# AlexZou14/Wave-Mamba

Hardware: AMD Instinct MI355X
Metric: UHD (3840x2160) images/sec fwd (higher is better)
Workload: dtype f32; 1 GPU; Wave-Mamba UHD-LL inference config (wf=32, n_l=[1,2,4], n_h=[1,1,2]), 1x3x2160x3840 reflect-padded to 2176x3840, seeded random init, one image per GPU per step, replicas (no collective); one forward at a time, its down-path high-frequency branches on side streams: True

## Files before the change

include/wavemamba_hip.h:

```cpp
#ifndef WAVEMAMBA_HIP_H
#define WAVEMAMBA_HIP_H

#include <stddef.h>
#include <stdint.h>

#ifdef __cplusplus
extern "C" {
#endif

#define WM_OK 0
#define WM_EINVAL (-1)
#define WM_ENULL (-2)
#define WM_EALIGN (-3)
#define WM_EWORKSPACE (-4)
#define WM_EUNSUPPORTED (-5)
#define WM_EHIP (-6)

#define WM_F32 0
#define WM_BF16 1

int wm_abi_version(void);
const char* wm_build_id(void);
const char* wm_strerror(int code);

// ... 55 lines not shown
                    const float* skip_scale2, float* out, int out_nchw, int B, int64_t L, int C, int plane_dtype,
                    void* stream);
int wm_lfss_in_conv_fwd(const float* tok, int tok_nchw, const float* ln_w, const float* ln_b, float ln_eps,
                        const float* in_proj_weight, const float* conv_weight, const float* conv_bias, float* xc,
                        int B, int H, int W, int C, int plane_dtype, void* stream);
int wm_lfss_in_conv_band_rows(int B, int H, int W);
int wm_lfss_out_conv_fwd(const void* f, const float* conv2_weight, const float* conv2_bias, const float* tok1,
                         const float* conv3_weight, const float* conv3_bias, const float* skip_scale2, float* out,
                         int out_nchw, int B, int H, int W, int C, int plane_dtype, void* stream);
int wm_lfss_mid_rz_tok_fwd(const void* ysum, int ny, int64_t ystride, const float* tok, int tok_nchw, const float* ln1_w,
                           const float* ln1_b, float ln1_eps, const float* in_proj_weight, const float* out_norm_w,
                           const float* out_norm_b, float out_norm_eps, const float* out_proj_weight, const float* skip_scale,
                           float* tok1, int B, int64_t L, int C, int plane_dtype, void* stream);
int wm_lfss_ffn_fwd(const float* tok1, const float* ln2_w, const float* ln2_b, float ln2_eps, const float* conv1_weight,
                    const float* conv1_bias, const float* conv2_weight, const float* conv2_bias, const float* conv3_weight,
                    const float* conv3_bias, const float* skip_scale2, float* out, int out_nchw, int B, int H, int W, int C,
                    int plane_dtype, int band_rows, void* stream);
int wm_lfss_ffn_band_rows(int B, int H, int W);

int wm_layernorm2d_fwd(const float* x, const float* weight, const float* bias, float eps, float* y,
                       int B, int64_t L, int C, void* stream);

size_t wm_gram_workspace_bytes(int B, int C, int64_t L);
int wm_gram_fwd(const float* X, const float* Y, float* G, float* nx, float* ny, void* workspace,
                size_t workspace_bytes, int B, int C, int64_t L, void* stream);

int wm_dwconv3x3_wgrad(const float* x, const float* gy, float* dW, float* db, int B, int C, int H, int W,
                       void* stream);
int wm_layernorm2d_bwd(const float* x, const float* weight, const float* gy, float eps, float* gx,
                       float* dweight, float* dbias, int B, int64_t L, int C, void* stream);


int wm_conv2d_select(int mode);
size_t wm_conv2d_wfrag_bytes(int Cout, int Cin, int ks);
int wm_conv2d_prep(const float* weight, void* wfrag, int Cout, int Cin, int ks, void* stream);
int wm_conv2d_ln_fwd(const float* x, const float* ln_weight, const float* ln_bias, float ln_eps, const void* wfrag, const float* bias,
                     const float* residual, float* y, int B, int Cin, int Cout, int H, int W, void* stream);
int wm_dwconv_conv1x1_fwd(const float* x, int64_t x_batch_stride, const float* dw_weight, const float* dw_bias, int act,
                          const void* wfrag, const float* bias, const float* residual, float* y, int B, int C, int Cout, int H,
                          int W, void* stream);
int wm_ln_conv1x1_dwconv_fwd(const float* x, const float* ln_weight, const float* ln_bias, float ln_eps, const void* wfrag,
                             const float* bias, const float* dw_weight, const float* dw_bias, float* y, int B, int Cin, int Cout,
                             int Cdw, int H, int W, int band_rows, void* stream);
int wm_conv2d_f16_steps(const float* x, const float* weight, const float* bias, float* y, float* amax, void* wfrag, int B, int Cin,
                        int Cout, int H, int W, int ks, int dgrad, void* stream);
int wm_conv2d_fwd(const float* xa, const float* xb, const int* xb_index, const void* wfrag, const float* bias,
                  const float* gate, const float* residual, float* y, int B, int Ca, int Cb, int Cb_src, int Cout,
                  int H, int W, int ks, void* stream);
int wm_conv2d_gated_fwd(const float* xa, const float* xb, const int* xb_index, const void* wfrag3, const void* wfrag1,
                        const float* bias1, float* y, int B, int Ca, int Cb, int Cb_src, int Cout, int H, int W,
                        void* stream);
int wm_conv2d_dwt_fwd(const void* img, const void* wfrag, const float* bias, void* ll, void* hl, void* lh, void* hh, int B, int Cin,
                      int Cout, int H, int W, int dtype, void* stream);
int wm_idwt_conv2d_fwd(const void* low, const void* high, const void* wfrag, const float* bias, const float* residual, float* y, int B,
                       int Cin, int Cout, int H, int W, int dtype, void* stream);

size_t wm_ss2d_core_bwd_workspace_bytes(int B, int D, int H, int W, int N, int R);
int wm_ss2d_core_bwd(const float* x, const float* x_proj_weight, const float* dt_projs_weight,
                     const float* dt_projs_bias, const float* A_logs, const float* Ds, const float* dy_row_fwd,
                     const float* dy_row_rev, const float* dy_col_fwd, const float* dy_col_rev, float* dx,
                     float* dx_proj_weight, float* ddt_projs_weight, float* ddt_projs_bias, float* dA_logs, float* dDs,
                     void* workspace, size_t workspace_bytes, int B, int D, int H, int W, int N, int R, void* stream);

int wm_layernorm_tok_fwd(const float* x, const float* weight, const float* bias, float eps, float* y, int64_t T, int C,
                         void* stream);
int wm_layernorm_tok_bwd(const float* x, const float* weight, const float* gy, float eps, float* gx, float* dweight,
// ... 90 lines not shown
```

wave_mamba_amd/_lib.py:

```python
import ctypes
import os

HERE = os.path.dirname(os.path.abspath(__file__))
LIB_PATH = os.environ.get("WAVEMAMBA_HIP_LIB") or os.path.join(HERE, "libwavemamba_hip.so")

WM_F32, WM_BF16 = 0, 1
WM_OK, WM_EINVAL, WM_ENULL, WM_EALIGN, WM_EWORKSPACE, WM_EUNSUPPORTED, WM_EHIP = 0, -1, -2, -3, -4, -5, -6
WM_PROF_NKERNELS = 20
ABI_VERSION = 34

_c = ctypes
_p, _i, _i64, _sz = _c.c_void_p, _c.c_int, _c.c_int64, _c.c_size_t

SIGNATURES = {
    "wm_abi_version": (_i, []),
    "wm_build_id": (_c.c_char_p, []),
    "wm_strerror": (_c.c_char_p, [_i]),
    "wm_dwt2d_fwd": (_i, [_p] * 5 + [_i] * 5 + [_p]),
    "wm_dwt2d_bwd": (_i, [_p] * 5 + [_i] * 5 + [_p]),
    "wm_idwt2d_fwd": (_i, [_p] * 4 + [_i64] * 4 + [_p] + [_i] * 5 + [_p]),
    "wm_idwt2d_bwd": (_i, [_p] * 5 + [_i64] * 4 + [_i] * 5 + [_p]),
    "wm_selscan_fwd_workspace_bytes": (_sz, [_i] * 5),
    "wm_selscan_fwd": (_i, [_p] * 10 + [_p, _sz] + [_i] * 6 + [_p]),
    "wm_selscan_bwd_workspace_bytes": (_sz, [_i] * 5),
# ... 31 lines not shown
    "wm_paired_patches_u8": (_i, [_p, _p, _p, _i, _i, _i, _p]),
    "wm_linear_wgrad": (_i, [_p, _p, _p, _i64, _i, _i, _p]),
    "wm_conv2d_wgrad_workspace_bytes": (_sz, [_i] * 6),
    "wm_conv2d_wgrad": (_i, [_p, _p, _p, _p, _p, _sz] + [_i] * 6 + [_p]),
    "wm_plane_sums": (_i, [_p, _p, _i, _i, _i, _i, _p]),
    "wm_psnr_ssim_y_workspace_bytes": (_sz, [_i] * 4),
    "wm_psnr_ssim_y_u8": (_i, [_p, _p] + [_i64] * 4 + [_i] * 5 + [_p, _p, _sz, _p]),
    "wm_y_channel_u8": (_i, [_p] + [_i64] * 4 + [_i] * 4 + [_p, _p]),
    "wm_l1_mean_fwd": (_i, [_p, _p, _p, _i64, _p]),
    "wm_l1_mean_bwd": (_i, [_p, _p, _p, _p, _i64, _p]),
    "wm_ssim_workspace_bytes": (_sz, [_i64, _i, _i]),
    "wm_ssim_mean_fwd": (_i, [_p] * 8 + [_sz, _i64, _i, _i, _p]),
    "wm_ssim_mean_bwd": (_i, [_p] * 7 + [_i64, _i, _i, _p]),
    "wm_gate_fwd": (_i, [_p] * 3 + [_i, _i] + [_i64] * 4 + [_p]),
    "wm_gate_bwd": (_i, [_p] * 5 + [_i, _i] + [_i64] * 6 + [_p]),
    "wm_scale_add_fwd": (_i, [_p] * 4 + [_i, _i, _i64, _p]),
    "wm_scale_add_bwd": (_i, [_p] * 5 + [_i, _i, _i64, _p]),
    "wm_match_index": (_i, [_p, _p, _p, _p, _i, _i, _p]),
    "wm_attn_fold": (_i, [_p] * 6 + [_i, _i, _i, _p]),
    "wm_skff_workspace_bytes": (_sz, [_i, _i]),
    "wm_skff_fwd": (_i, [_p] * 7 + [_p, _sz] + [_i] * 5 + [_p]),
    "wm_conv2d_wfrag_bytes": (_sz, [_i, _i, _i]),
    "wm_conv2d_prep": (_i, [_p, _p, _i, _i, _i, _p]),
    "wm_conv2d_fwd": (_i, [_p] * 8 + [_i] * 8 + [_p]),
    "wm_conv2d_ln_fwd": (_i, [_p, _p, _p, _c.c_float, _p, _p, _p, _p] + [_i] * 5 + [_p]),
    "wm_dwconv_conv1x1_fwd": (_i, [_p, _i64, _p, _p, _i, _p, _p, _p, _p] + [_i] * 5 + [_p]),
    "wm_ln_conv1x1_dwconv_fwd": (_i, [_p, _p, _p, _c.c_float, _p, _p, _p, _p, _p] + [_i] * 7 + [_p]),
    "wm_patchify_conv_fwd": (_i, [_p] * 4 + [_i] * 6 + [_p]),
    "wm_conv2d_f16_steps": (_i, [_p] * 6 + [_i] * 7 + [_p]),
    "wm_conv2d_gated_fwd": (_i, [_p] * 7 + [_i] * 7 + [_p]),
    "wm_conv2d_dwt_fwd": (_i, [_p] * 7 + [_i] * 6 + [_p]),
    "wm_idwt_conv2d_fwd": (_i, [_p] * 6 + [_i] * 6 + [_p]),
    "wm_conv2d_select": (_i, [_i]),
    "wm_prof_enable": (None, [ctypes.c_uint]),
    "wm_prof_collect": (_i, [_c.POINTER(_i), _c.POINTER(_c.c_double)]),
    "wm_event_synchronize_relaxed": (_i, [_p]),
    "wm_zero_arena_register": (_i, [_p, _c.c_size_t]),
    "wm_zero_arena_unregister": (_i, [_p]),
    "wm_dwconv3x3_wgrad_det_workspace_bytes": (_sz, [_i] * 4),
    "wm_dwconv3x3_wgrad_det": (_i, [_p] * 4 + [_p, _sz] + [_i] * 4 + [_p]),
    "wm_layernorm2d_bwd_det_workspace_bytes": (_sz, [_i, _i64, _i]),
    "wm_layernorm2d_bwd_det": (_i, [_p, _p, _p, _c.c_float, _p, _p, _p, _p, _sz, _i, _i64, _i, _p]),
    "wm_layernorm_tok_bwd_det_workspace_bytes": (_sz, [_i64, _i]),
    "wm_layernorm_tok_bwd_det": (_i, [_p, _p, _p, _c.c_float, _p, _p, _p, _p, _sz, _i64, _i, _p]),
    "wm_linear_wgrad_det_workspace_bytes": (_sz, [_i64, _i, _i]),
    "wm_linear_wgrad_det": (_i, [_p, _p, _p, _p, _sz, _i64, _i, _i, _p]),
    "wm_plane_sums_det_workspace_bytes": (_sz, [_i] * 4),
    "wm_plane_sums_det": (_i, [_p, _p, _p, _sz, _i, _i, _i, _i, _p]),
    "wm_scale_add_bwd_det_workspace_bytes": (_sz, [_i, _i, _i64]),
    "wm_scale_add_bwd_det": (_i, [_p] * 5 + [_p, _sz, _i, _i, _i64, _p]),
    "wm_l1_mean_fwd_det_workspace_bytes": (_sz, [_i64]),
    "wm_l1_mean_fwd_det": (_i, [_p, _p, _p, _p, _sz, _i64, _p]),
    "wm_selscan_bwd_det_workspace_bytes": (_sz, [_i] * 5),
    "wm_selscan_bwd_det": (_i, [_p] * 15 + [_p, _sz] + [_i] * 6 + [_p]),
    "wm_channel_gather_fwd": (_i, [_p, _p, _p, _i, _i, _i, _i64, _p]),
    "wm_channel_gather_bwd": (_i, [_p, _p, _p, _i, _i, _i, _i64, _p]),
}

_lib = None


class WaveMambaHipError(RuntimeError):
    pass


def load():
# ... 36 lines not shown
```

wave_mamba_amd/csrc/conv.hip:

```cpp
#include "host_common.h"
#include "conv2d.hip.h"
#include "conv2d_ws.hip.h"
#include "patchify.hip.h"
#include "dw_pw.hip.h"
#include "pw_dw.hip.h"

using namespace wm;

static Conv2dArgs conv_args(const void* xa, int Ca, const void* wfrag, const float* bias, void* y, int Cout, int H, int W) {
    Conv2dArgs a;
    a.xa = (const float*)xa; a.wfrag = (const uint4*)wfrag; a.bias = bias; a.y = (float*)y;
    a.Ca = Ca; a.Cout = Cout; a.H = H; a.W = W;
    a.nch = (Ca + 15) / 16; a.mtot = (Cout + 31) / 32;
    return a;
}

static int conv_tail_check(int B, int H, int W, const void* wfrag) {
    if (B > 65535 || (long long)H * W >= (1ll << 31)) return WM_EUNSUPPORTED;
    if (!aligned16(wfrag)) return WM_EALIGN;
    return WM_OK;
}

template <int KS, int RW, int MT, bool G1X1 = false, bool F16 = false, bool LNIN = false>
static int conv2d_launch(const wm::Conv2dArgs& a, int B, hipStream_t st) {
// ... 11 lines not shown
}

#ifndef WM_CONV_WS_RW2
#define WM_CONV_WS_RW2 4
#endif
#ifndef WM_CONV_WS_RW1
#define WM_CONV_WS_RW1 4
#endif
#ifndef WM_CONV_WS_RWG
#define WM_CONV_WS_RWG 2
#endif
#ifndef WM_CONV_WS_NPW1
#define WM_CONV_WS_NPW1 4
#endif
#ifndef WM_CONV_RW1
#define WM_CONV_RW1 3
#endif
static std::atomic<int> g_conv_select{0};
static int conv_select_mode() { return g_conv_select.load(std::memory_order_relaxed); }
static long long conv_ws_ntiles(const wm::Conv2dArgs& a, int B, int th) {
    return (long long)B * ((a.W + wm::kWsTW - 1) / wm::kWsTW) * ((a.H + th - 1) / th);
}
static bool conv_ws_enabled(const wm::Conv2dArgs& a, int B, int th) {
    const int mode = conv_select_mode();
    if (mode == 1) return false;
    const long long cmax = std::max(std::max(a.Ca, a.xb ? a.Cbsrc : 0), a.Cout);
    if (cmax * a.H * a.W * 4 >= (1ll << 32) || (a.xb_idx && a.Cb > 128)) return false;
    if (a.gate && a.res) return false;
    if (mode == 2) return true;
    if ((a.gate || a.res) && a.mtot > 1) return false;
    return conv_ws_ntiles(a, B, th) >= 768;
}

template <int RW, int MT, bool G1X1 = false, bool EPI = false, int NPW = 4, bool F16 = false, bool DWTE = false, bool IWTI = false>
static int conv2d_ws_launch(const wm::Conv2dArgs& a, int B, hipStream_t st) {
    using Cfg = wm::ConvWsCfg<RW, MT, G1X1, NPW>;
    static bool configured[64] = {};
    int ncu = 0;
    int rc = wm::lds_optin((const void*)wm::conv3x3_ws_kernel<RW, MT, G1X1, EPI, NPW, F16, DWTE, IWTI>, Cfg::LDS_BYTES, configured);
    if (!rc) rc = wm::device_cus(&ncu);
    if (rc) return rc;
    const long long ntiles = conv_ws_ntiles(a, B, Cfg::TH);
    if (ntiles >= (1ll << 31)) return WM_EUNSUPPORTED;
    const int cus = std::max(8, ncu & ~7);
    const int G = (int)std::min<long long>(cus, ((ntiles + 7) / 8) * 8);
    hipLaunchKernelGGL((wm::conv3x3_ws_kernel<RW, MT, G1X1, EPI, NPW, F16, DWTE, IWTI>), dim3((unsigned)G), dim3(256 + 64 * NPW), Cfg::LDS_BYTES, st, a, B);
    return launch_status();
}

template <bool F16, bool LNIN>
static int conv2d_walk(wm::Conv2dArgs& a, int B, int ks, hipStream_t st) {
    for (int mb = 0, n; mb < a.mtot; mb += n) {
        a.mbase = mb;
        const int left = a.mtot - mb;
        int rc = WM_EUNSUPPORTED;
        n = 1;
        if (LNIN || ks == 1) {
            if (left >= 3) { rc = conv2d_launch<1, 2, 3, false, F16, LNIN>(a, B, st); n = 3; }
            else if (left == 2) { rc = conv2d_launch<1, 4, 2, false, F16, LNIN>(a, B, st); n = 2; }
            else rc = conv2d_launch<1, 4, 1, false, F16, LNIN>(a, B, st);
        } else if constexpr (!LNIN) {
            if (conv_ws_enabled(a, B, 8)) {
                const bool epi = !F16 && (a.gate || a.res);
                if (epi) { if constexpr (!F16) rc = conv2d_ws_launch<WM_CONV_WS_RW1, 1, false, true>(a, B, st); }
                else if (left >= 2) { rc = conv2d_ws_launch<WM_CONV_WS_RW2, 2, false, false, 4, F16>(a, B, st); n = 2; }
                else rc = conv2d_ws_launch<WM_CONV_WS_RW1, 1, false, false, WM_CONV_WS_NPW1, F16>(a, B, st);
            } else if (left >= 2) { rc = conv2d_launch<3, 4, 2, false, F16>(a, B, st); n = 2; }
            else rc = conv2d_launch<3, WM_CONV_RW1, 1, false, F16>(a, B, st);
        }
        if (rc) return rc;
    }
    return WM_OK;
}

extern "C" {

int wm_patchify_conv_fwd(const float* img, const float* weight, const float* bias, float* y, int B, int Cin, int Cout, int H, int W,
                         int r, void* stream) {
    if (B < 0 || Cin <= 0 || Cout <= 0 || H < 0 || W < 0) return WM_EINVAL;
    if (r != 2 && r != 4 && r != 8) return WM_EUNSUPPORTED;
    if (H % r || W % r) return WM_EINVAL;
    if (Cout != 16 && Cout != 32 && Cout != 48 && Cout != 64) return WM_EUNSUPPORTED;
    const size_t lds = (size_t)Cin * r * r * Cout * sizeof(float);
    if (lds > 64 * 1024) return WM_EUNSUPPORTED;
    if (B == 0 || H == 0 || W == 0) return WM_OK;
    if (!img || !weight || !y) return WM_ENULL;
    if (!aligned16(img)) return WM_EALIGN;
    if ((long long)B * Cin * H * W >= (1ll << 40)) return WM_EUNSUPPORTED;
    const int Ho = H / r, Wo = W / r;
    const int spr = (Wo + 255) / 256;
    const long long nsegs = (long long)B * Ho * spr;
    const int spb = (int)((nsegs + 4095) / 4096);
    const long long blocks = (nsegs + spb - 1) / spb;
    hipStream_t st = (hipStream_t)stream;
    ProfScope ps(18, st);
#define WM_PF(R, CO) hipLaunchKernelGGL((patchify_conv_kernel<R, CO>), dim3((unsigned)blocks), dim3(256), lds, st, img, weight, bias, y, \
                                        B, Cin, H, W, spr, nsegs, spb)
#define WM_PFR(R) do { if (Cout == 16) WM_PF(R, 16); else if (Cout == 32) WM_PF(R, 32); else if (Cout == 48) WM_PF(R, 48); else WM_PF(R, 64); } while (0)
    if (r == 2) WM_PFR(2); else if (r == 4) WM_PFR(4); else WM_PFR(8);
// ... 135 lines not shown
    if (ks != 1 && ks != 3) return WM_EUNSUPPORTED;
    if (wm_conv2d_wfrag_bytes(Cout, Cin, ks) == 0) return WM_EUNSUPPORTED;
    if (B == 0 || H == 0 || W == 0) return WM_OK;
    if (!x || !weight || !y || !amax || !wfrag) return WM_ENULL;
    if (!aligned16(wfrag)) return WM_EALIGN;
    hipStream_t st = (hipStream_t)stream;
    if (zero_out(amax, 2 * sizeof(float), st) != hipSuccess) return WM_EHIP;
    const long long nx = (long long)B * Cin * H * W, nw = (long long)Cout * Cin * ks * ks;
    long long blocks = (nx / 4 + 256 * 8 - 1) / (256 * 8);
    blocks = blocks < 1 ? 1 : (blocks > 512 ? 512 : blocks);
    const int nch = (Cin + 15) / 16, mtot = (Cout + 31) / 32;
    const long long items = (long long)nch * ks * ks * mtot * 128;
    const int nprep = (int)(items <= 512 ? 1 : (items >= 32 * 512 ? 32 : (items + 511) / 512));
    hipLaunchKernelGGL(cv_amax_prep_kernel, dim3((unsigned)blocks + nprep), dim3(256), 0, st, x, nx, weight, nw, (unsigned*)amax,
                       (uint4*)wfrag, Cout, Cin, ks * ks, nch, mtot, dgrad ? 1 : 0, nprep);
    int rc = launch_status();
    if (rc) return rc;
    return conv2d_fwd_f16(x, wfrag, amax, bias, y, B, Cin, Cout, H, W, ks, stream);
}

int wm_conv2d_dwt_fwd(const void* img, const void* wfrag, const float* bias, void* ll, void* hl, void* lh, void* hh, int B, int Cin,
                      int Cout, int H, int W, int dtype, void* stream) {
    if (B < 0 || Cin <= 0 || Cout <= 0 || H < 0 || W < 0) return WM_EINVAL;
    if (H % 2 || W % 2) return WM_EINVAL;
    if (dtype != WM_F32 || Cout != 32) return WM_EUNSUPPORTED;
    if (B == 0 || H == 0 || W == 0) return WM_OK;
    if (!img || !wfrag || !ll || !hl || !lh || !hh) return WM_ENULL;
    if (const int rc = conv_tail_check(B, H, W, wfrag)) return rc;
    hipStream_t st = (hipStream_t)stream;
    Conv2dArgs a = conv_args(img, Cin, wfrag, bias, ll, Cout, H, W);
    a.yband[0] = (float*)hl; a.yband[1] = (float*)lh; a.yband[2] = (float*)hh;
    if (conv_select_mode() == 1 || (long long)std::max(Cin, Cout) * H * W * 4 >= (1ll << 32)) return WM_EUNSUPPORTED;
    ProfScope ps(13, st);
    return conv2d_ws_launch<WM_CONV_WS_RW1, 1, false, false, WM_CONV_WS_NPW1, false, true>(a, B, st);
}

int wm_idwt_conv2d_fwd(const void* low, const void* high, const void* wfrag, const float* bias, const float* residual, float* y, int B,
                       int Cin, int Cout, int H, int W, int dtype, void* stream) {
    if (B < 0 || Cin <= 0 || Cout <= 0 || H < 0 || W < 0) return WM_EINVAL;
    if (H % 2 || W % 2) return WM_EINVAL;
    if (dtype != WM_F32 || Cin != 32) return WM_EUNSUPPORTED;
    if (B == 0 || H == 0 || W == 0) return WM_OK;
    if (!low || !high || !wfrag || !y) return WM_ENULL;
    if (const int rc = conv_tail_check(B, H, W, wfrag)) return rc;
    hipStream_t st = (hipStream_t)stream;
    Conv2dArgs a = conv_args(low, Cin, wfrag, bias, y, Cout, H, W);
    a.xb = (const float*)high; a.Cbsrc = 3 * Cin;
    a.res = residual;
    if (conv_select_mode() == 1 || (long long)std::max(Cin, Cout) * H * W * 4 >= (1ll << 32)) return WM_EUNSUPPORTED;
    ProfScope ps(13, st);
    for (int mb = 0; mb < a.mtot; ++mb) {
        a.mbase = mb;
        const int rc = residual ? conv2d_ws_launch<WM_CONV_WS_RW1, 1, false, true, 4, false, false, true>(a, B, st)
                                : conv2d_ws_launch<WM_CONV_WS_RW1, 1, false, false, WM_CONV_WS_NPW1, false, false, true>(a, B, st);
        if (rc) return rc;
    }
    return WM_OK;
}

int wm_conv2d_gated_fwd(const float* xa, const float* xb, const int* xb_index, const void* wfrag3, const void* wfrag1,
                        const float* bias1, float* y, int B, int Ca, int Cb, int Cb_src, int Cout, int H, int W,
                        void* stream) {
    if (B < 0 || Ca <= 0 || Cb < 0 || Cout <= 0 || H < 0 || W < 0 || Cb_src < 0) return WM_EINVAL;
    if (B == 0 || H == 0 || W == 0) return WM_OK;
    if (!xa || !wfrag3 || !wfrag1 || !y || (Cb > 0 && !xb)) return WM_ENULL;
    if (Cb > 0 && Ca % 8 != 0) return WM_EUNSUPPORTED;
    if (Cb > 0 && !xb_index && Cb_src != Cb) return WM_EINVAL;
    if (const int rc = conv_tail_check(B, H, W, wfrag3)) return rc;
    if (!aligned16(wfrag1)) return WM_EALIGN;
    hipStream_t st = (hipStream_t)stream;
    Conv2dArgs a = conv_args(xa, Ca, wfrag3, nullptr, y, Cout, H, W);
    if (Cb > 0) { a.xb = xb; a.xb_idx = xb_index; }
    a.Cb = Cb; a.Cbsrc = Cb_src; a.nch = (Ca + Cb + 15) / 16;
    a.wfrag1 = (const uint4*)wfrag1; a.bias1 = bias1;
    ProfScope ps(13, st);
    for (int mb = 0; mb < a.mtot;) {
        a.mbase = mb;
        int rc;
        const bool two = a.mtot - mb >= 2;
        if (conv_ws_enabled(a, B, two ? 2 * WM_CONV_WS_RWG : 8)) {
            if (two) { rc = conv2d_ws_launch<WM_CONV_WS_RWG, 2, true>(a, B, st); mb += 2; }
            else { rc = conv2d_ws_launch<4, 1, true>(a, B, st); mb += 1; }
        } else if (a.mtot - mb >= 2) { rc = conv2d_launch<3, 2, 2, true>(a, B, st); mb += 2; }
        else { rc = conv2d_launch<3, 4, 1, true>(a, B, st); mb += 1; }
        if (rc) return rc;
    }
    return WM_OK;
}

int wm_conv2d_select(int mode) {
    if (mode < 0 || mode > 2) return WM_EINVAL;
    g_conv_select.store(mode, std::memory_order_relaxed);
    return WM_OK;
}

#if WM_CV_STAMP
int wm_debug_conv_stamps(unsigned long long* out) {
    return (int)hipMemcpyFromSymbol(out, HIP_SYMBOL(wm::g_cv_stamps), sizeof(unsigned long long) * 2 * 128 * 8);
}
#endif

}
```

wave_mamba_amd/csrc/conv2d_ws.hip.h:

```cpp
#pragma once
#include <type_traits>
#include "conv2d.hip.h"
#include "haar.hip.h"

namespace wm {

constexpr int kWsTW = 64;

template <int RW, int MT, bool G1X1, int NPW = 4>
struct ConvWsCfg {
    static constexpr int NPT = 64 * NPW;
    static constexpr int PW = kWsTW + 2;
    static constexpr int TH = 2 * RW;
    static constexpr int NPIX = (TH + 2) * PW;
    static constexpr int PIT = (NPIX + NPT - 1) / NPT;
    static constexpr int W_ITEMS = 9 * MT * 2 * 64;
    static constexpr int W1_ITEMS = G1X1 ? MT * 2 * 64 : 0;
    static constexpr int BUF_ITEMS = 4 * NPIX + W_ITEMS + W1_ITEMS;
    static constexpr int LDS_BYTES = 2 * BUF_ITEMS * 16 + 2 * MT * 32 * 4;
};

struct ConvWsTiles {
    int tiles_x, ntiles_img, first, stride, count;
    __device__ ConvWsTiles(int B, int H, int W, int TH, int g, int G) {
        tiles_x = (W + kWsTW - 1) / kWsTW;
        ntiles_img = tiles_x * ((H + TH - 1) / TH);
        const int ntiles = ntiles_img * B, nper = (ntiles + 7) / 8;
        const int x = g & 7, slot = g >> 3;
        stride = G >> 3;
        first = x * nper + slot;
        const int end = min((x + 1) * nper, ntiles);
        count = first < end ? (end - first + stride - 1) / stride : 0;
    }
    __device__ void locate(int j, int TH, int& b, int& h0, int& w0) const {
        const int t = first + j * stride;
        b = t / ntiles_img;
        const int ti = t - b * ntiles_img;
        h0 = (ti / tiles_x) * TH;
        w0 = (ti % tiles_x) * kWsTW;
    }
};

#ifndef WM_CV_STAMP
#define WM_CV_STAMP 0
#endif
#if WM_CV_STAMP
__device__ unsigned long long g_cv_stamps[2 * 128 * 8];
#define CV_STAMP(role, it, k) do { if (WM_CV_STAMP && blockIdx.x == 0 && lane == 0 && (wave & 3) == 0 && (it) < 128) \
        g_cv_stamps[((role) * 128 + (it)) * 8 + (k)] = __builtin_readcyclecounter(); } while (0)
#else
#define CV_STAMP(role, it, k) do { } while (0)
#endif

using u32x4_t = __attribute__((ext_vector_type(4))) unsigned;
template <int OFF>
__device__ __forceinline__ void ws_lds_store16(unsigned addr, const uint4& v) {
    u32x4_t d = {v.x, v.y, v.z, v.w};
    asm volatile("ds_write_b128 %0, %1 offset:%2" : : "v"(addr), "v"(d), "n"(OFF) : "memory");
}

__device__ __forceinline__ void ws_barrier_lds() { asm volatile("s_waitcnt lgkmcnt(0)\n\ts_barrier" ::: "memory"); }

__device__ __forceinline__ float ws_from_pair_lane(float v) {
    return __builtin_bit_cast(float, __builtin_amdgcn_update_dpp(0, __builtin_bit_cast(int, v), 0xB1, 0xf, 0xf, false));
}

template <int RW, int MT, bool G1X1, bool EPI, int NPW = 4, bool F16 = false, bool DWTE = false, bool IWTI = false>
__global__ __launch_bounds__(256 + 64 * NPW, (4 + NPW) / 4) void conv3x3_ws_kernel(const Conv2dArgs a, const int B) {
    extern __shared__ __attribute__((aligned(16))) unsigned char cv_smem[];
    static_assert(!(F16 && G1X1), "the fp16 form (conv2d.hip.h) serves the plain convolutions of the training step");
    static_assert(!DWTE || (MT == 1 && !G1X1 && !EPI && !F16 && RW % 2 == 0), "the analysis epilogue: one plain 32-channel row tile, whole quads per wave");
    static_assert(!IWTI || (!G1X1 && !F16), "the synthesis staging: the plain bf16 form");
    const float sx = F16 ? cv_pow2_scale(a.amax[0]) : 1.0f;
    const float osc = F16 ? 1.0f / (sx * cv_pow2_scale(a.amax[1])) : 1.0f;
    using Cfg = ConvWsCfg<RW, MT, G1X1, NPW>;
    constexpr int PW = Cfg::PW, TH = Cfg::TH, NPIX = Cfg::NPIX, PIT = Cfg::PIT, NPT = Cfg::NPT;
    constexpr int W_ITEMS = Cfg::W_ITEMS, W1_ITEMS = Cfg::W1_ITEMS, BUF = Cfg::BUF_ITEMS;
    uint4* const smem = reinterpret_cast<uint4*>(cv_smem);

    const int tid = threadIdx.x, lane = tid & 63;
    const int wave = __builtin_amdgcn_readfirstlane(tid >> 6);
    const ConvWsTiles tl(B, a.H, a.W, TH, (int)blockIdx.x, (int)gridDim.x);
    if (tl.count == 0) return;
    const int nch = a.nch;
    const int n_it = tl.count * nch;
    const int H = a.H, W = a.W;
    const long long HW = (long long)H * W;

    if (tid < 2 * MT * 32) {
        const int which = tid / (MT * 32), ch = a.mbase * 32 + tid % (MT * 32);
        const float* src = which ? a.bias1 : a.bias;
        reinterpret_cast<float*>(smem + 2 * BUF)[tid] = (src && ch < a.Cout) ? src[ch] : 0.0f;
    }
    if (wave >= 4) {
        const int ptid = tid - 256, pw = wave - 4;
        const unsigned lds_base = (unsigned)(size_t)(__attribute__((address_space(3))) unsigned char*)cv_smem;
        static_assert(2 * NPIX * 16 < 65536, "the lo plane sits within the ds_write offset field");
        constexpr int QR = (TH + 4) / 2, QC = (kWsTW + 4) / 2;
        static_assert(!IWTI || QR * QC <= NPT, "one quad per producer thread");
        constexpr int PSL = IWTI ? 4 : PIT;
        const int qr = IWTI ? ptid / QC : 0, qc = IWTI ? ptid - qr * QC : 0;
        const int h2 = IWTI ? a.H >> 1 : 0, w2 = IWTI ? a.W >> 1 : 0;
        const unsigned HW2b = IWTI ? (unsigned)(h2 * w2) * 4u : 0u;
        float pin[2][2][PSL][8];
        unsigned okm[2][PIT];
        int ccs[2] = {0, 0};
        unsigned poff[PIT];
        unsigned okF[PIT];
        int jf = -1, ccf = nch - 1;
        const float* xaF = a.xa;
        const float* xbF = a.xa;
        int idxv0 = 0, idxv1 = 0, bF = -1;

        auto fetch_w = [&](int buf, int cc) {
            uint4* s_w = smem + buf * BUF + 4 * NPIX;
            const uint4* wsrc = a.wfrag + ((long long)cc * 9 * a.mtot) * 128;
            constexpr int W_IT = (W_ITEMS + NPT - 1) / NPT;
#pragma unroll
            for (int it = 0; it < W_IT; ++it) {
                const int item0 = it * NPT + pw * 64;
                if (W_ITEMS % NPT == 0 || item0 < W_ITEMS) {
                    const int tm = item0 >> 7, tap = tm / MT, m = tm - tap * MT;
                    const uint4* g = wsrc + (tap * a.mtot + a.mbase + m) * 128 + (item0 & 64) + lane;
                    __builtin_amdgcn_global_load_lds((const __attribute__((address_space(1))) void*)g,
                                                     (__attribute__((address_space(3))) void*)(s_w + item0), 16, 0, 0);
                }
            }
            if constexpr (G1X1) {
// ... 143 lines not shown
            ws_barrier_lds();
            CV_STAMP(1, i, 4);
        };

        advance(); fetch_half(C0{}, C0{}); fetch_half(C0{}, C1{});
        fetch_w(0, ccs[0]);
        if (n_it > 1) { advance(); fetch_half(C1{}, C0{}); fetch_half(C1{}, C1{}); }
        stage_half(C0{}, C0{}, 0); stage_half(C0{}, C1{}, 0);
        __builtin_amdgcn_s_waitcnt(0x0070);
        ws_barrier_lds();
        for (int i = 0; i < n_it; i += 2) {
            step(C0{}, C1{}, i + 2 < n_it, i + 1 < n_it, 1, i);
            if (i + 1 >= n_it) break;
            step(C1{}, C0{}, i + 3 < n_it, i + 2 < n_it, 0, i + 1);
        }
        return;
    }

    f32x16_t acc[MT][RW];
    f32x16_t acc1[G1X1 ? MT : 1][G1X1 ? RW : 1];
    auto zero_acc = [&](auto MC) {
        constexpr int m = decltype(MC)::value;
#pragma unroll
        for (int r = 0; r < RW; ++r)
#pragma unroll
            for (int i = 0; i < 16; ++i) { acc[m][r][i] = 0.0f; if (G1X1) acc1[m][r][i] = 0.0f; }
    };
    using M0 = std::integral_constant<int, 0>;
    using M1 = std::integral_constant<int, MT - 1>;
    static_assert(MT <= 2, "at most two row tiles per launch");
    zero_acc(M0{});
    if (MT > 1) zero_acc(M1{});
    const int khalf = lane >> 5, px = lane & 31;
    const int cw = wave & 1, rg = wave >> 1;

    const bool full = (a.mbase + MT) * 32 <= a.Cout;
    const float* s_bias = reinterpret_cast<const float*>(smem + 2 * BUF);
    const unsigned HWb = (unsigned)HW * 4u;
    auto tile_fast = [&](int j, int& b, int& h0, int& w0) {
        tl.locate(j, TH, b, h0, w0);
        return full && h0 + TH <= H && w0 + kWsTW <= W;
    };

    auto mma = [&](int buf) {
        const uint4* s_in = smem + buf * BUF;
        const uint4* s_w = s_in + 4 * NPIX;
        const uint4* s_w1 = s_w + W_ITEMS;
#pragma unroll
        for (int kx = 0; kx < 3; ++kx) {
            Frag16 Ah[3][MT], Al[3][MT];
#pragma unroll
            for (int ky = 0; ky < 3; ++ky)
#pragma unroll
                for (int m = 0; m < MT; ++m) {
                    Ah[ky][m].u = s_w[(((ky * 3 + kx) * MT + m) * 2 + 0) * 64 + lane];
                    Al[ky][m].u = s_w[(((ky * 3 + kx) * MT + m) * 2 + 1) * 64 + lane];
                }
#pragma unroll
            for (int j = 0; j < RW + 2; ++j) {
                const int pidx = (rg * RW + j) * PW + cw * 32 + px + kx;
                Frag16 Bh, Bl;
                Bh.u = s_in[khalf * NPIX + pidx];
                Bl.u = s_in[(2 + khalf) * NPIX + pidx];
#pragma unroll
                for (int term = 0; term < 3; ++term)
#pragma unroll
                    for (int ky = 0; ky < 3; ++ky) {
// ... 78 lines not shown
                for (int i = 0; i < 16; ++i) {
                    const int dc = (i & 3) + 8 * (i >> 2);
                    const bool ok = in && (full || chb + dc < a.Cout);
                    ev[r][i] = ok ? eptr[o + dc * HW] : 0.0f;
                }
            }
        }
        {
            const int chb = (a.mbase + m) * 32 + 4 * khalf;
            float bv[16], b1v[G1X1 ? 16 : 1];
#pragma unroll
            for (int i = 0; i < 16; ++i) {
                const int cl = m * 32 + 4 * khalf + (i & 3) + 8 * (i >> 2);
                bv[i] = s_bias[cl];
                if (G1X1) b1v[i] = s_bias[MT * 32 + cl];
            }
#pragma unroll
            for (int r = 0; r < RW; ++r) {
                const int h = h0 + rg * RW + r;
                if (h >= H || w >= W) continue;
                const long long o = (((long long)b * a.Cout + chb) * H + h) * W + w;
#pragma unroll
                for (int i = 0; i < 16; ++i) {
                    const int dc = (i & 3) + 8 * (i >> 2);
                    float v = (F16 ? acc[m][r][i] * osc : acc[m][r][i]) + bv[i];
                    if constexpr (G1X1) v = v / (1.0f + __expf(-(acc1[m][r][i] + b1v[i])));
                    if constexpr (EPI) v = is_gate ? v / (1.0f + __expf(-ev[r][i])) : v + ev[r][i];
                    if (full || chb + dc < a.Cout) a.y[o + dc * HW] = v;
                }
            }
        }
    };

    auto epilogue_dwt = [&](int j) {
        int b, h0, w0;
        const bool fast = tile_fast(j, b, h0, w0);
        const int w = w0 + cw * 32 + px, hq = (h0 + rg * RW) >> 1;
        const bool odd = px & 1;
        const int h2 = H >> 1, w2 = W >> 1;
        const unsigned HW2b = (unsigned)(h2 * w2) * 4u;
        const size_t bo = (size_t)b * a.Cout * HW2b;
        char* const y0 = reinterpret_cast<char*>(odd ? a.yband[1] : a.y) + bo;
        char* const y1 = reinterpret_cast<char*>(odd ? a.yband[2] : a.yband[0]) + bo;
        const int chb = a.mbase * 32 + 4 * khalf;
        const unsigned o0 = (unsigned)((chb * h2 + hq) * w2 + (w >> 1)) * 4u;
        float bv[16];
#pragma unroll
        for (int i = 0; i < 16; ++i) bv[i] = s_bias[4 * khalf + (i & 3) + 8 * (i >> 2)];
        auto quads = [&](auto FASTC) {
            constexpr bool FAST = decltype(FASTC)::value;
#pragma unroll
            for (int rp = 0; rp < RW / 2; ++rp) {
                const bool in = FAST || (h0 + rg * RW + 2 * rp < H && w < W);
#pragma unroll
                for (int i = 0; i < 16; ++i) {
                    const int dc = (i & 3) + 8 * (i >> 2);
                    const float v0 = acc[0][2 * rp][i] + bv[i], v1 = acc[0][2 * rp + 1][i] + bv[i];
                    const float n0 = ws_from_pair_lane(v0), n1 = ws_from_pair_lane(v1);
                    float ll, hl, lh, hh;
                    haar_fwd<false>(odd ? n0 : v0, odd ? n1 : v1, odd ? v0 : n0, odd ? v1 : n1, ll, hl, lh, hh);
                    const unsigned o = o0 + (unsigned)(rp * w2) * 4u + (unsigned)dc * HW2b;
                    if (FAST || (in && (full || chb + dc < a.Cout))) {
                        *reinterpret_cast<float*>(y0 + (size_t)o) = odd ? lh : ll;
                        *reinterpret_cast<float*>(y1 + (size_t)o) = odd ? hh : hl;
                    }
                }
            }
        };
        if (fast) quads(std::true_type{});
        else quads(std::false_type{});
    };

    ws_barrier_lds();
    int cc = 0, j = 0;
    for (int i = 0; i < n_it; ++i) {
        CV_STAMP(0, i, 0);
        mma(i & 1);
        CV_STAMP(0, i, 1);
        ws_barrier_lds();
        CV_STAMP(0, i, 2);
        if (++cc == nch) {
            if constexpr (DWTE) epilogue_dwt(j);
            else {
                epilogue(j, M0{});
                if (MT > 1) epilogue(j, M1{});
            }
            zero_acc(M0{});
            if (MT > 1) zero_acc(M1{});
            cc = 0; ++j;
        }
        CV_STAMP(0, i, 3);
    }
}

}
```

Before: 36.44 images/s.

## Add two alternating consumer wave groups to overlap conv epilogue with MMA

The warp-specialized 3x3 conv kernel can now run two groups of four consumer waves that take output tiles in turn. While one group runs the MMA for its tile, the other writes out its previous tile's epilogue in slices spread over the chunk iterations, so store traffic overlaps compute. Producer waves get raised scheduling priority in this mode. It applies to the plain single-tile f32 form and the DWT-fused analysis conv, chosen by a tile-count heuristic or a runtime override, at the cost of larger blocks and fewer registers per wave.

```diff
diff --git a/include/wavemamba_hip.h b/include/wavemamba_hip.h
--- a/include/wavemamba_hip.h
+++ b/include/wavemamba_hip.h
@@ -111,6 +111,7 @@
 
 
 int wm_conv2d_select(int mode);
+int wm_conv2d_ws_groups(int mode);
 size_t wm_conv2d_wfrag_bytes(int Cout, int Cin, int ks);
 int wm_conv2d_prep(const float* weight, void* wfrag, int Cout, int Cin, int ks, void* stream);
 int wm_conv2d_ln_fwd(const float* x, const float* ln_weight, const float* ln_bias, float ln_eps, const void* wfrag, const float* bias,
diff --git a/wave_mamba_amd/_lib.py b/wave_mamba_amd/_lib.py
--- a/wave_mamba_amd/_lib.py
+++ b/wave_mamba_amd/_lib.py
@@ -87,6 +87,7 @@
     "wm_conv2d_dwt_fwd": (_i, [_p] * 7 + [_i] * 6 + [_p]),
     "wm_idwt_conv2d_fwd": (_i, [_p] * 6 + [_i] * 6 + [_p]),
     "wm_conv2d_select": (_i, [_i]),
+    "wm_conv2d_ws_groups": (_i, [_i]),
     "wm_prof_enable": (None, [ctypes.c_uint]),
     "wm_prof_collect": (_i, [_c.POINTER(_i), _c.POINTER(_c.c_double)]),
     "wm_event_synchronize_relaxed": (_i, [_p]),
diff --git a/wave_mamba_amd/csrc/conv.hip b/wave_mamba_amd/csrc/conv.hip
--- a/wave_mamba_amd/csrc/conv.hip
+++ b/wave_mamba_amd/csrc/conv.hip
@@ -67,19 +67,31 @@
     return conv_ws_ntiles(a, B, th) >= 768;
 }
 
-template <int RW, int MT, bool G1X1 = false, bool EPI = false, int NPW = 4, bool F16 = false, bool DWTE = false, bool IWTI = false>
+static std::atomic<int> g_conv_ws_groups{0};
+static bool conv_ws_two_groups(const wm::Conv2dArgs& a, long long ntiles, int G) {
+    const int mode = g_conv_ws_groups.load(std::memory_order_relaxed);
+    if (mode) return mode == 2;
+    return (a.nch == 1 || a.nch >= 4) && ntiles / G >= 15;
+}
+
+template <int RW, int MT, bool G1X1 = false, bool EPI = false, int NPW = 4, bool F16 = false, bool DWTE = false, bool IWTI = false, int NCG = 1>
 static int conv2d_ws_launch(const wm::Conv2dArgs& a, int B, hipStream_t st) {
     using Cfg = wm::ConvWsCfg<RW, MT, G1X1, NPW>;
-    static bool configured[64] = {};
     int ncu = 0;
-    int rc = wm::lds_optin((const void*)wm::conv3x3_ws_kernel<RW, MT, G1X1, EPI, NPW, F16, DWTE, IWTI>, Cfg::LDS_BYTES, configured);
-    if (!rc) rc = wm::device_cus(&ncu);
+    int rc = wm::device_cus(&ncu);
     if (rc) return rc;
     const long long ntiles = conv_ws_ntiles(a, B, Cfg::TH);
     if (ntiles >= (1ll << 31)) return WM_EUNSUPPORTED;
     const int cus = std::max(8, ncu & ~7);
     const int G = (int)std::min<long long>(cus, ((ntiles + 7) / 8) * 8);
-    hipLaunchKernelGGL((wm::conv3x3_ws_kernel<RW, MT, G1X1, EPI, NPW, F16, DWTE, IWTI>), dim3((unsigned)G), dim3(256 + 64 * NPW), Cfg::LDS_BYTES, st, a, B);
+    if constexpr (NCG == 2) {
+        if (!conv_ws_two_groups(a, ntiles, G)) return conv2d_ws_launch<RW, MT, G1X1, EPI, NPW, F16, DWTE, IWTI, 1>(a, B, st);
+    }
+    static bool configured[64] = {};
+    rc = wm::lds_optin((const void*)wm::conv3x3_ws_kernel<RW, MT, G1X1, EPI, NPW, F16, DWTE, IWTI, NCG>, Cfg::LDS_BYTES, configured);
+    if (rc) return rc;
+    hipLaunchKernelGGL((wm::conv3x3_ws_kernel<RW, MT, G1X1, EPI, NPW, F16, DWTE, IWTI, NCG>), dim3((unsigned)G), dim3(64 * (4 * NCG + NPW)),
+                       Cfg::LDS_BYTES, st, a, B);
     return launch_status();
 }
 
@@ -99,7 +111,7 @@
                 const bool epi = !F16 && (a.gate || a.res);
                 if (epi) { if constexpr (!F16) rc = conv2d_ws_launch<WM_CONV_WS_RW1, 1, false, true>(a, B, st); }
                 else if (left >= 2) { rc = conv2d_ws_launch<WM_CONV_WS_RW2, 2, false, false, 4, F16>(a, B, st); n = 2; }
-                else rc = conv2d_ws_launch<WM_CONV_WS_RW1, 1, false, false, WM_CONV_WS_NPW1, F16>(a, B, st);
+                else rc = conv2d_ws_launch<WM_CONV_WS_RW1, 1, false, false, WM_CONV_WS_NPW1, F16, false, false, F16 ? 1 : 2>(a, B, st);
             } else if (left >= 2) { rc = conv2d_launch<3, 4, 2, false, F16>(a, B, st); n = 2; }
             else rc = conv2d_launch<3, WM_CONV_RW1, 1, false, F16>(a, B, st);
         }
@@ -301,7 +313,7 @@
     a.yband[0] = (float*)hl; a.yband[1] = (float*)lh; a.yband[2] = (float*)hh;
     if (conv_select_mode() == 1 || (long long)std::max(Cin, Cout) * H * W * 4 >= (1ll << 32)) return WM_EUNSUPPORTED;
     ProfScope ps(13, st);
-    return conv2d_ws_launch<WM_CONV_WS_RW1, 1, false, false, WM_CONV_WS_NPW1, false, true>(a, B, st);
+    return conv2d_ws_launch<WM_CONV_WS_RW1, 1, false, false, WM_CONV_WS_NPW1, false, true, false, 2>(a, B, st);
 }
 
 int wm_idwt_conv2d_fwd(const void* low, const void* high, const void* wfrag, const float* bias, const float* residual, float* y, int B,
@@ -363,10 +375,16 @@
     return WM_OK;
 }
 
+int wm_conv2d_ws_groups(int mode) {
+    if (mode < 0 || mode > 2) return WM_EINVAL;
+    g_conv_ws_groups.store(mode, std::memory_order_relaxed);
+    return WM_OK;
+}
+
 #if WM_CV_STAMP
 int wm_debug_conv_stamps(unsigned long long* out) {
-    return (int)hipMemcpyFromSymbol(out, HIP_SYMBOL(wm::g_cv_stamps), sizeof(unsigned long long) * 2 * 128 * 8);
-}
-#endif
-
-}
+    return (int)hipMemcpyFromSymbol(out, HIP_SYMBOL(wm::g_cv_stamps), sizeof(unsigned long long) * 3 * 128 * 8);
+}
+#endif
+
+}
diff --git a/wave_mamba_amd/csrc/conv2d_ws.hip.h b/wave_mamba_amd/csrc/conv2d_ws.hip.h
--- a/wave_mamba_amd/csrc/conv2d_ws.hip.h
+++ b/wave_mamba_amd/csrc/conv2d_ws.hip.h
@@ -45,7 +45,7 @@
 #define WM_CV_STAMP 0
 #endif
 #if WM_CV_STAMP
-__device__ unsigned long long g_cv_stamps[2 * 128 * 8];
+__device__ unsigned long long g_cv_stamps[3 * 128 * 8];
 #define CV_STAMP(role, it, k) do { if (WM_CV_STAMP && blockIdx.x == 0 && lane == 0 && (wave & 3) == 0 && (it) < 128) \
         g_cv_stamps[((role) * 128 + (it)) * 8 + (k)] = __builtin_readcyclecounter(); } while (0)
 #else
@@ -65,12 +65,14 @@
     return __builtin_bit_cast(float, __builtin_amdgcn_update_dpp(0, __builtin_bit_cast(int, v), 0xB1, 0xf, 0xf, false));
 }
 
-template <int RW, int MT, bool G1X1, bool EPI, int NPW = 4, bool F16 = false, bool DWTE = false, bool IWTI = false>
-__global__ __launch_bounds__(256 + 64 * NPW, (4 + NPW) / 4) void conv3x3_ws_kernel(const Conv2dArgs a, const int B) {
+template <int RW, int MT, bool G1X1, bool EPI, int NPW = 4, bool F16 = false, bool DWTE = false, bool IWTI = false, int NCG = 1>
+__global__ __launch_bounds__(64 * (4 * NCG + NPW), (4 * NCG + NPW) / 4) void conv3x3_ws_kernel(const Conv2dArgs a, const int B) {
     extern __shared__ __attribute__((aligned(16))) unsigned char cv_smem[];
     static_assert(!(F16 && G1X1), "the fp16 form (conv2d.hip.h) serves the plain convolutions of the training step");
     static_assert(!DWTE || (MT == 1 && !G1X1 && !EPI && !F16 && RW % 2 == 0), "the analysis epilogue: one plain 32-channel row tile, whole quads per wave");
     static_assert(!IWTI || (!G1X1 && !F16), "the synthesis staging: the plain bf16 form");
+    static_assert(NCG == 1 || (NCG == 2 && MT == 1 && !G1X1 && !EPI && !F16 && !IWTI), "two consumer groups: the forms that fit 168 registers (DESIGN.md 4)");
+    constexpr int NCW = 4 * NCG;
     const float sx = F16 ? cv_pow2_scale(a.amax[0]) : 1.0f;
     const float osc = F16 ? 1.0f / (sx * cv_pow2_scale(a.amax[1])) : 1.0f;
     using Cfg = ConvWsCfg<RW, MT, G1X1, NPW>;
@@ -92,8 +94,9 @@
         const float* src = which ? a.bias1 : a.bias;
         reinterpret_cast<float*>(smem + 2 * BUF)[tid] = (src && ch < a.Cout) ? src[ch] : 0.0f;
     }
-    if (wave >= 4) {
-        const int ptid = tid - 256, pw = wave - 4;
+    if (wave >= NCW) {
+        const int ptid = tid - 64 * NCW, pw = wave - NCW;
+        if (NCG == 2) __builtin_amdgcn_s_setprio(3);
         const unsigned lds_base = (unsigned)(size_t)(__attribute__((address_space(3))) unsigned char*)cv_smem;
         static_assert(2 * NPIX * 16 < 65536, "the lo plane sits within the ds_write offset field");
         constexpr int QR = (TH + 4) / 2, QC = (kWsTW + 4) / 2;
@@ -303,7 +306,8 @@
     zero_acc(M0{});
     if (MT > 1) zero_acc(M1{});
     const int khalf = lane >> 5, px = lane & 31;
-    const int cw = wave & 1, rg = wave >> 1;
+    const int cw = wave & 1, rg = (wave >> 1) & 1;
+    const int grp = wave >> 2;
 
     const bool full = (a.mbase + MT) * 32 <= a.Cout;
     const float* s_bias = reinterpret_cast<const float*>(smem + 2 * BUF);
@@ -448,9 +452,29 @@
         }
     };
 
-    auto epilogue_dwt = [&](int j) {
-        int b, h0, w0;
-        const bool fast = tile_fast(j, b, h0, w0);
+    constexpr int NU = DWTE ? RW / 2 : RW;
+    auto epi_walk = [&](auto FASTC, int b, int h0, int w0, int lo, int hi) {
+        constexpr bool FAST = decltype(FASTC)::value;
+        const int w = w0 + cw * 32 + px, hb = h0 + rg * RW;
+        char* const yb = reinterpret_cast<char*>(a.y) + (size_t)b * a.Cout * HW * 4;
+        const int chb = a.mbase * 32 + 4 * khalf;
+        const unsigned o0 = ((unsigned)(chb * H + hb) * (unsigned)W + (unsigned)w) * 4u;
+#pragma unroll
+        for (int r = 0; r < RW; ++r) {
+            if (r < lo || r >= hi) continue;
+            const bool in = FAST || (hb + r < H && w < W);
+#pragma unroll
+            for (int i = 0; i < 16; ++i) {
+                const int dc = (i & 3) + 8 * (i >> 2);
+                const float v = acc[0][r][i] + s_bias[4 * khalf + dc];
+                const unsigned o = o0 + (unsigned)(r * W) * 4u + (unsigned)dc * HWb;
+                if (FAST || (in && (full || chb + dc < a.Cout))) *reinterpret_cast<float*>(yb + (size_t)o) = v;
+            }
+        }
+    };
+
+    auto epi_walk_dwt = [&](auto FASTC, int b, int h0, int w0, int lo, int hi) {
+        constexpr bool FAST = decltype(FASTC)::value;
         const int w = w0 + cw * 32 + px, hq = (h0 + rg * RW) >> 1;
         const bool odd = px & 1;
         const int h2 = H >> 1, w2 = W >> 1;
@@ -460,52 +484,83 @@
         char* const y1 = reinterpret_cast<char*>(odd ? a.yband[2] : a.yband[0]) + bo;
         const int chb = a.mbase * 32 + 4 * khalf;
         const unsigned o0 = (unsigned)((chb * h2 + hq) * w2 + (w >> 1)) * 4u;
-        float bv[16];
-#pragma unroll
-        for (int i = 0; i < 16; ++i) bv[i] = s_bias[4 * khalf + (i & 3) + 8 * (i >> 2)];
-        auto quads = [&](auto FASTC) {
-            constexpr bool FAST = decltype(FASTC)::value;
-#pragma unroll
-            for (int rp = 0; rp < RW / 2; ++rp) {
-                const bool in = FAST || (h0 + rg * RW + 2 * rp < H && w < W);
-#pragma unroll
-                for (int i = 0; i < 16; ++i) {
-                    const int dc = (i & 3) + 8 * (i >> 2);
-                    const float v0 = acc[0][2 * rp][i] + bv[i], v1 = acc[0][2 * rp + 1][i] + bv[i];
-                    const float n0 = ws_from_pair_lane(v0), n1 = ws_from_pair_lane(v1);
-                    float ll, hl, lh, hh;
-                    haar_fwd<false>(odd ? n0 : v0, odd ? n1 : v1, odd ? v0 : n0, odd ? v1 : n1, ll, hl, lh, hh);
-                    const unsigned o = o0 + (unsigned)(rp * w2) * 4u + (unsigned)dc * HW2b;
-                    if (FAST || (in && (full || chb + dc < a.Cout))) {
-                        *reinterpret_cast<float*>(y0 + (size_t)o) = odd ? lh : ll;
-                        *reinterpret_cast<float*>(y1 + (size_t)o) = odd ? hh : hl;
-                    }
-                }
-            }
-        };
-        if (fast) quads(std::true_type{});
-        else quads(std::false_type{});
+#pragma unroll
+        for (int rp = 0; rp < RW / 2; ++rp) {
+            if (rp < lo || rp >= hi) continue;
+            const bool in = FAST || (h0 + rg * RW + 2 * rp < H && w < W);
+#pragma unroll
+            for (int i = 0; i < 16; ++i) {
+                const int dc = (i & 3) + 8 * (i >> 2);
+                const float bv = s_bias[4 * khalf + dc];
+                const float v0 = acc[0][2 * rp][i] + bv, v1 = acc[0][2 * rp + 1][i] + bv;
+                const float n0 = ws_from_pair_lane(v0), n1 = ws_from_pair_lane(v1);
+                float ll, hl, lh, hh;
+                haar_fwd<false>(odd ? n0 : v0, odd ? n1 : v1, odd ? v0 : n0, odd ? v1 : n1, ll, hl, lh, hh);
+                const unsigned o = o0 + (unsigned)(rp * w2) * 4u + (unsigned)dc * HW2b;
+                if (FAST || (in && (full || chb + dc < a.Cout))) {
+                    *reinterpret_cast<float*>(y0 + (size_t)o) = odd ? lh : ll;
+                    *reinterpret_cast<float*>(y1 + (size_t)o) = odd ? hh : hl;
+                }
+            }
+        }
+    };
+    auto epi_units = [&](int j, int lo, int hi) {
+        int b, h0, w0;
+        const bool fast = tile_fast(j, b, h0, w0);
+        if constexpr (DWTE) {
+            if (fast) epi_walk_dwt(std::true_type{}, b, h0, w0, lo, hi);
+            else epi_walk_dwt(std::false_type{}, b, h0, w0, lo, hi);
+        } else if constexpr (NCG == 2) {
+            if (fast) epi_walk(std::true_type{}, b, h0, w0, lo, hi);
+            else epi_walk(std::false_type{}, b, h0, w0, lo, hi);
+        }
+    };
+    auto zero_all = [&]() {
+        zero_acc(M0{});
+        if (MT > 1) zero_acc(M1{});
     };
 
     ws_barrier_lds();
-    int cc = 0, j = 0;
-    for (int i = 0; i < n_it; ++i) {
-        CV_STAMP(0, i, 0);
-        mma(i & 1);
-        CV_STAMP(0, i, 1);
-        ws_barrier_lds();
-        CV_STAMP(0, i, 2);
-        if (++cc == nch) {
-            if constexpr (DWTE) epilogue_dwt(j);
-            else {
-                epilogue(j, M0{});
-                if (MT > 1) epilogue(j, M1{});
-            }
-            zero_acc(M0{});
-            if (MT > 1) zero_acc(M1{});
-            cc = 0; ++j;
-        }
-        CV_STAMP(0, i, 3);
+    if constexpr (NCG == 1) {
+        int cc = 0, j = 0;
+        for (int i = 0; i < n_it; ++i) {
+            CV_STAMP(0, i, 0);
+            mma(i & 1);
+            CV_STAMP(0, i, 1);
+            ws_barrier_lds();
+            CV_STAMP(0, i, 2);
+            if (++cc == nch) {
+                if constexpr (DWTE) epi_units(j, 0, NU);
+                else {
+                    epilogue(j, M0{});
+                    if (MT > 1) epilogue(j, M1{});
+                }
+                zero_all();
+                cc = 0; ++j;
+            }
+            CV_STAMP(0, i, 3);
+        }
+    } else {
+        const int srole = grp ? 2 : 0;
+        int cc = 0, jt = 0, pend = -1;
+        for (int i = 0; i <= n_it; ++i) {
+            const bool mine = i < n_it && (jt & 1) == grp;
+            CV_STAMP(srole, i, 0);
+            if (mine) mma(i & 1);
+            else if (pend >= 0) {
+                const int lo = i < n_it ? cc * NU / nch : 0, hi = i < n_it ? (cc + 1) * NU / nch : NU;
+                epi_units(pend, lo, hi);
+                if (hi == NU) { zero_all(); pend = -1; }
+            }
+            CV_STAMP(srole, i, 1);
+            if (i == n_it) break;
+            ws_barrier_lds();
+            CV_STAMP(srole, i, 2);
+            if (++cc == nch) {
+                if (mine) pend = jt;
+                cc = 0; ++jt;
+            }
+        }
     }
 }
 
```

Result: no change. 36.48 images/s, median of 3 (+0.1%).
